# AsherJingkongChen/vlm-bridge-for-image-captioning

Hardware: NVIDIA B200
Metric: bridge fwd+bwd samples/sec (higher is better)
Workload: dtype bf16

## Files before the change

vlm-bridge-for-image-captioning_b200/csrc/attention.cu:

```cuda
#include <math.h>
#include <stdlib.h>
#include <string.h>

#include "common.cuh"
#include "launch.h"

namespace b200b {

int attention_fwd_tc(const b200b_attn_args* a, cudaStream_t stream, int* taken);
int attention_bwd_tc(const b200b_attn_args* a, const float* delta, cudaStream_t stream, int* taken);

struct AttnParams {
  const __nv_bfloat16* q; long long ldq;
  const __nv_bfloat16* k; long long ldk;
  const __nv_bfloat16* v; long long ldv;
  __nv_bfloat16* o; long long ldo;
  const __nv_bfloat16* d_o; long long lddo;
  __nv_bfloat16* dq; long long lddq;
  __nv_bfloat16* dk; long long lddk;
  __nv_bfloat16* dv; long long lddv;
  float* lse2;
  float* delta;
  __nv_bfloat16* p_scr;
  __nv_bfloat16* ds_scr;
  int B, H, Lq, Lk, Lkp;
  long long kv_bstride, kv_hstride;
  float scale, scale_log2;
  DropoutCfg drop;
  uint32_t drop_stream;
};

template <int HD>
struct AttnCfg {
  static constexpr int kBM = 64;
  static constexpr int kBN = (HD > 128) ? 32 : 64;
  static constexpr int kLd = HD + 8;
  static constexpr int kRowBytes = HD * 2;
  static constexpr int kQT = 32;
  static constexpr int kScrLd = 40;
  static constexpr size_t kFwdSmem = (size_t)(kBM + 4 * kBN) * kLd * 2;
  static constexpr size_t kBwdQSmem = (size_t)(2 * kBM + 4 * kBN) * kLd * 2;
  static constexpr size_t kBwdKVSmem = (size_t)2 * (2 * kQT * kScrLd + 2 * kQT * kLd) * 2;
};
// ... 468 lines not shown
    if (row0 < p.Lq) p.lse2[bh * p.Lq + row0] = m_run[0] + log2f(l_run[0]);
    if (row0 + 8 < p.Lq) p.lse2[bh * p.Lq + row0 + 8] = m_run[1] + log2f(l_run[1]);
  }
  {
    const float s0 = 1.0f / l_run[0], s1 = 1.0f / l_run[1];
    __nv_bfloat16* stage = Qs + (size_t)rg * 16 * kLd + half * (HD / 2);
#pragma unroll
    for (int n = 0; n < NH; ++n) {
      *reinterpret_cast<uint32_t*>(stage + (size_t)g * kLd + n * 8 + 2 * t4) = pack_bf16(o_acc[n][0] * s0, o_acc[n][1] * s0);
      *reinterpret_cast<uint32_t*>(stage + (size_t)(g + 8) * kLd + n * 8 + 2 * t4) =
          pack_bf16(o_acc[n][2] * s1, o_acc[n][3] * s1);
    }
    __syncwarp();
    const int rows_valid = max(0, min(16, nq - rg * 16));
    constexpr int kChunks = HD / 16;
    __nv_bfloat16* gdst = p.o + ((size_t)b * p.Lq + q0 + rg * 16) * p.ldo + (size_t)h * HD + half * (HD / 2);
    for (int idx = lane; idx < 16 * kChunks; idx += 32) {
      const int r = idx / kChunks, c = idx % kChunks;
      if (r < rows_valid)
        *reinterpret_cast<uint4*>(gdst + (size_t)r * p.ldo + c * 8) = *reinterpret_cast<const uint4*>(stage + (size_t)r * kLd + c * 8);
    }
  }
}

__global__ void attn_delta_kernel(const __nv_bfloat16* __restrict__ o, long long ldo,
                                  const __nv_bfloat16* __restrict__ d_o, long long lddo, float* __restrict__ delta,
                                  int B, int H, int Lq, int HD) {
  pdl_prologue();
  const int warp = threadIdx.x >> 5, lane = threadIdx.x & 31;
  const long long row = blockIdx.x;
  if (warp >= H) return;
  const uint32_t* po = reinterpret_cast<const uint32_t*>(o + row * ldo + (size_t)warp * HD);
  const uint32_t* pd = reinterpret_cast<const uint32_t*>(d_o + row * lddo + (size_t)warp * HD);
  float s = 0.f;
  for (int c = lane; c < HD / 2; c += 32) {
    const uint32_t a = po[c], d = pd[c];
    s += bf16_lo(a) * bf16_lo(d) + bf16_hi(a) * bf16_hi(d);
  }
  s = warp_sum(s);
  if (lane == 0) {
    const long long b = row / Lq, i = row % Lq;
    delta[((size_t)b * H + warp) * Lq + i] = s;
  }
}

template <int HD>
__global__ void __launch_bounds__(128) attn_bwd_q_kernel(const AttnParams p) {
  pdl_prologue();
  const DropoutCfg drop = dropout_resolve(p.drop);
  using Cfg = AttnCfg<HD>;
  constexpr int BN = Cfg::kBN, kLd = Cfg::kLd;
  extern __shared__ __align__(16) uint8_t smem_attn[];
  __nv_bfloat16* Qs = reinterpret_cast<__nv_bfloat16*>(smem_attn);
  __nv_bfloat16* dOs = Qs + (size_t)Cfg::kBM * kLd;
  __nv_bfloat16* Ks = dOs + (size_t)Cfg::kBM * kLd;
  __nv_bfloat16* Vs = Ks + (size_t)2 * BN * kLd;
  __shared__ __align__(8) uint64_t qbar, full_bar[2];

  const int warp = threadIdx.x >> 5, lane = threadIdx.x & 31;
  const int b = blockIdx.z, h = blockIdx.y, q0 = blockIdx.x * Cfg::kBM;
  const int nq = min(Cfg::kBM, p.Lq - q0);
  const int nt = (p.Lk + BN - 1) / BN;

  if (threadIdx.x == 0) {
    mbar_init(&qbar, 1);
    mbar_init(&full_bar[0], 1);
    mbar_init(&full_bar[1], 1);
    fence_barrier_init();
  }
  __syncthreads();
  if (warp == 0) {
    if (lane == 0) mbar_arrive_expect_tx(&qbar, (uint32_t)(2 * nq * Cfg::kRowBytes));
// ... 202 lines not shown
  launch_pdl(kPdlAttn, attn_fwd_kernel<HD>, grid, dim3(128), Cfg::kFwdSmem, stream, p);
  return check_launch("attn_fwd", stream);
}

static bool use_decode_kernel(const AttnParams& p) { return p.drop.thr == 0 && p.Lq <= 64; }

template <int HD, bool PACKED>
static int launch_decode(const AttnParams& p, cudaStream_t stream) {
  using Cfg = DecodeCfg<HD>;
  static bool attr_done = false;
  if (!attr_done) {
    int rc = set_smem(attn_decode_kernel<HD, PACKED>, Cfg::smem_bytes(2), "attn_decode");
    if (rc) return rc;
    attr_done = true;
  }
  const int nrg = (min(64, p.Lq) + 15) / 16;
  dim3 grid((p.Lq + 63) / 64, p.H, p.B);
  AttnParams pp = p;
#ifdef B200B_DIAG
  static const int dbg = [] { const char* e = getenv("B200B_DECODE_DEBUG"); return e ? atoi(e) : 0; }();
  if (dbg & 1) pp.Lkp = -1;
#endif
  launch_pdl(kPdlAttn, attn_decode_kernel<HD, PACKED>, grid, dim3(256), Cfg::smem_bytes(nrg), stream, pp);
  return check_launch(PACKED ? "attn_decode_packed" : "attn_decode", stream);
}

template <int HD>
static int launch_bwd(const AttnParams& p, cudaStream_t stream, const b200b_attn_args* a) {
  using Cfg = AttnCfg<HD>;
  int rc = set_smem(attn_bwd_q_kernel<HD>, Cfg::kBwdQSmem, "attn_bwd_q");
  if (rc) return rc;
  rc = set_smem(attn_bwd_kv_kernel<HD>, Cfg::kBwdKVSmem, "attn_bwd_kv");
  if (rc) return rc;
  const int delta_threads = 32 * p.H;
  launch_pdl(kPdlAttn, attn_delta_kernel, dim3(p.B * p.Lq), dim3(delta_threads), 0, stream, p.o, p.ldo, p.d_o, p.lddo, p.delta, p.B, p.H, p.Lq,
             HD);
  rc = check_launch("attn_delta", stream);
  if (rc) return rc;
  {
    int taken = 0;
    rc = attention_bwd_tc(a, p.delta, stream, &taken);
    if (taken) return rc;
  }
  dim3 gq((p.Lq + Cfg::kBM - 1) / Cfg::kBM, p.H, p.B);
  launch_pdl(kPdlAttn, attn_bwd_q_kernel<HD>, gq, dim3(128), Cfg::kBwdQSmem, stream, p);
  rc = check_launch("attn_bwd_q", stream);
  if (rc) return rc;
  dim3 gk((p.Lk + 31) / 32, p.H, p.B);
  launch_pdl(kPdlAttn, attn_bwd_kv_kernel<HD>, gk, dim3(128), Cfg::kBwdKVSmem, stream, p);
  return check_launch("attn_bwd_kv", stream);
}

static bool al16p(const void* p) { return (reinterpret_cast<uintptr_t>(p) & 15) == 0; }

static int validate_common(const b200b_attn_args* a, const char* what) {
  if (a == nullptr || !a->q || !a->k || !a->v || !a->o || !a->lse) {
    set_last_error("%s: null argument", what);
    return B200B_ERR_ARG;
  }
  if (a->batch <= 0 || a->heads <= 0 || a->heads > 32 || a->len_q <= 0 || a->len_k <= 0) {
    set_last_error("%s: bad sizes (batch=%d heads=%d len_q=%d len_k=%d)", what, a->batch, a->heads, a->len_q, a->len_k);
    return B200B_ERR_SHAPE;
  }
  if (a->head_dim != 64 && a->head_dim != 128 && a->head_dim != 288) {
    set_last_error("%s: head_dim %d not built (64, 128, 288)", what, a->head_dim);
    return B200B_ERR_SHAPE;
  }
  if (!al16p(a->q) || !al16p(a->k) || !al16p(a->v) || !al16p(a->o) || (a->ldq % 8) || (a->ldk % 8) || (a->ldv % 8) ||
      (a->ldo % 8)) {
    set_last_error("%s: q/k/v/o must be 16-byte aligned with row pitch multiple of 8 elements", what);
    return B200B_ERR_ALIGN;
  }
  if (!(a->dropout_p >= 0.0f && a->dropout_p < 1.0f)) {
    set_last_error("%s: dropout_p must be in [0,1)", what);
    return B200B_ERR_ARG;
  }
// ... 173 lines not shown
```

vlm-bridge-for-image-captioning_b200/csrc/attention_train_tc.cu:

```cuda
#include <stdlib.h>
#include <string.h>

#include "../../include/b200_bridge.h"
#include "common.cuh"
#include "launch.h"

namespace b200b {

struct FwdTcParams {
  __nv_bfloat16* o; long long ldo;
  float* lse2;
  int B, H, Lq, Lk, Lkp;
  float scale_log2;
  DropoutCfg drop;
  uint32_t drop_stream;
};

int attn_tc_mask();

constexpr int kFBM = 128;
constexpr int kFBN = 64;
constexpr int kFThreads = 192;

template <int HD>
// ... 235 lines not shown
  if (!attr_done) {
    cudaError_t e = cudaFuncSetAttribute(attn_fwd_tc_kernel<HD>, cudaFuncAttributeMaxDynamicSharedMemorySize,
                                         (int)Cfg::kSmemBytes);
    if (e != cudaSuccess) {
      set_last_error("attention_fwd (tcgen05): cudaFuncSetAttribute failed: %s", cudaGetErrorString(e));
      return (int)e;
    }
    attr_done = true;
  }
  CUtensorMap tq, tk, tv;
  int rc = make_tmap_heads_sw64(&tq, a->q, a->ldq, HD, a->heads, a->len_q, a->batch, kFBM);
  if (rc != B200B_OK) return rc;
  rc = make_tmap_heads_sw64(&tk, a->k, a->ldk, HD, a->heads, a->len_k, a->batch, kFBN);
  if (rc != B200B_OK) return rc;
  rc = make_tmap_heads_sw64(&tv, a->v, a->ldv, HD, a->heads, a->len_k, a->batch, kFBN);
  if (rc != B200B_OK) return rc;
  FwdTcParams p;
  p.o = reinterpret_cast<__nv_bfloat16*>(a->o);
  p.ldo = a->ldo;
  p.lse2 = a->lse;
  p.B = a->batch; p.H = a->heads; p.Lq = a->len_q; p.Lk = a->len_k; p.Lkp = (a->len_k + 7) & ~7;
  p.scale_log2 = 1.4426950408889634f / sqrtf((float)HD);
  p.drop_stream = a->dropout_stream;
  p.drop = make_dropout_cfg(a->dropout_p, a->seed, &p.drop_stream);
  dim3 grid((a->len_q + kFBM - 1) / kFBM, a->heads, a->batch);
  launch_pdl(kPdlAttn, attn_fwd_tc_kernel<HD>, grid, dim3(kFThreads), Cfg::kSmemBytes, stream, tq, tk, tv, p);
  return check_launch("attn_fwd_tc", stream);
}

struct BwdTcParams {
  __nv_bfloat16* dq; long long lddq;
  __nv_bfloat16* dk; long long lddk;
  __nv_bfloat16* dv; long long lddv;
  const float* lse2;
  const float* delta;
  int B, H, Lq, Lk, Lkp;
  float scale, scale_log2;
  DropoutCfg drop;
  uint32_t drop_stream;
};

template <int HD>
struct DqTcCfg {
  static constexpr int kChunks = HD / 32;
  static constexpr int kQBytes = kFBM * HD * 2;
  static constexpr int kTileBytes = kFBN * HD * 2;
  static constexpr int kN0 = HD > 256 ? 160 : HD;
  static constexpr int kN1 = HD - kN0;
  static constexpr int kSCol = 0;
  static constexpr int kDpCol = kFBN;
  static constexpr int kDsCol = 2 * kFBN;
  static constexpr int kDqCol = 3 * kFBN;
  static constexpr uint32_t kTmemCols = (kDqCol + HD) <= 256 ? 256 : 512;
  static constexpr size_t kSmemBytes = 2 * (size_t)kQBytes + 2 * (size_t)kTileBytes + 1024;
};

template <int HD>
__global__ void __launch_bounds__(kFThreads, 1)
attn_bwd_dq_tc_kernel(const __grid_constant__ CUtensorMap tm_q, const __grid_constant__ CUtensorMap tm_do,
                      const __grid_constant__ CUtensorMap tm_k, const __grid_constant__ CUtensorMap tm_v,
                      const BwdTcParams p) {
  using Cfg = DqTcCfg<HD>;
  extern __shared__ uint8_t smem_ftc_raw[];
  __shared__ __align__(8) uint64_t qdo_full, k_full, k_free, v_full, v_free, s_full, ds_full, dq_done[2];
  __shared__ uint32_t tmem_base_smem;

  const int warp = threadIdx.x >> 5, lane = threadIdx.x & 31;
  const int q0 = blockIdx.x * kFBM, h = blockIdx.y, b = blockIdx.z;
  const uint32_t s0 = (smem_u32(smem_ftc_raw) + 1023u) & ~1023u;
  const uint32_t q_tile = s0, do_tile = s0 + Cfg::kQBytes;
  const uint32_t k_tile = do_tile + Cfg::kQBytes, v_tile = k_tile + Cfg::kTileBytes;
  const int nt = (p.Lk + kFBN - 1) / kFBN;

  if (threadIdx.x == 0) {
    mbar_init(&qdo_full, 1);
    mbar_init(&k_full, 1);
    mbar_init(&k_free, 1);
    mbar_init(&v_full, 1);
    mbar_init(&v_free, 1);
    mbar_init(&s_full, 1);
    mbar_init(&ds_full, 4);
    mbar_init(&dq_done[0], 1);
    mbar_init(&dq_done[1], 1);
    fence_barrier_init();
  }
  if (warp == 0) {
    tmem_alloc(&tmem_base_smem, Cfg::kTmemCols);
    tmem_relinquish();
  }
  if (warp == 5 && lane == 0) {
    tma_prefetch_desc(&tm_q);
    tma_prefetch_desc(&tm_do);
    tma_prefetch_desc(&tm_k);
    tma_prefetch_desc(&tm_v);
  }
  pdl_launch_dependents();
  pdl_wait();
  tc_fence_before();
  __syncthreads();
  tc_fence_after();
  const uint32_t tmem_base = tmem_base_smem;
// ... 34 lines not shown
          umma_bf16(tmem_base + Cfg::kSCol, desc_sw64_kmajor(q_tile, kFBM, ks), desc_sw64_kmajor(k_tile, kFBN, ks), idesc_s,
                    ks > 0);
        mbar_wait(&v_full, ph);
        tc_fence_after();
#pragma unroll
        for (int ks = 0; ks < HD / 16; ++ks)
          umma_bf16(tmem_base + Cfg::kDpCol, desc_sw64_kmajor(do_tile, kFBM, ks), desc_sw64_kmajor(v_tile, kFBN, ks),
                    idesc_s, ks > 0);
        umma_commit(&s_full);
        umma_commit(&v_free);
        mbar_wait(&ds_full, ph);
        tc_fence_after();
        const uint32_t da = tmem_base + (uint32_t)(Cfg::kDsCol + (t & 1) * (kFBN / 2));
        const uint32_t dd = tmem_base + (uint32_t)Cfg::kDqCol;
#pragma unroll
        for (int kc = 0; kc < kFBN / 16; ++kc) {
          umma_bf16_tmem_a(dd, da + (uint32_t)(kc * 8), desc_sw64_mnmajor(k_tile, kFBN, 0, kc), idesc_q0, (t | kc) != 0);
          if constexpr (Cfg::kN1 > 0)
            umma_bf16_tmem_a(dd + (uint32_t)Cfg::kN0, da + (uint32_t)(kc * 8),
                             desc_sw64_mnmajor(k_tile, kFBN, Cfg::kN0 / 32, kc), idesc_q1, (t | kc) != 0);
        }
        umma_commit(&dq_done[t & 1]);
        umma_commit(&k_free);
      }
    }
  } else {
    const DropoutCfg drop = dropout_resolve(p.drop);
    const int row = warp * 32 + lane;
    const bool valid = q0 + row < p.Lq;
    const uint32_t lane_off = (uint32_t)(warp * 32) << 16;
    const size_t bh = (size_t)b * p.H + h;
    const uint64_t ridx = (bh * p.Lq + (uint64_t)(q0 + row)) * (uint64_t)p.Lkp;
    const float lse = valid ? p.lse2[bh * p.Lq + q0 + row] : 0.f;
    const float del = valid ? p.delta[bh * p.Lq + q0 + row] : 0.f;
    for (int t = 0; t < nt; ++t) {
      mbar_wait(&s_full, (uint32_t)(t & 1));
      tc_fence_after();
      if (t >= 2) mbar_wait(&dq_done[t & 1], (uint32_t)(((t >> 1) - 1) & 1));
      tc_fence_after();
#pragma unroll
      for (int half = 0; half < kFBN / 32; ++half) {
        uint32_t sv[2][16], dv[2][16];
#pragma unroll
        for (int g = 0; g < 2; ++g) {
          tmem_ld_32x32_x16(tmem_base + lane_off + (uint32_t)(Cfg::kSCol + half * 32 + g * 16), sv[g]);
          tmem_ld_32x32_x16(tmem_base + lane_off + (uint32_t)(Cfg::kDpCol + half * 32 + g * 16), dv[g]);
        }
        tmem_ld_wait();
        uint32_t w[16];
#pragma unroll
        for (int g = 0; g < 2; ++g) {
          float ds[16];
#pragma unroll
          for (int j8 = 0; j8 < 2; ++j8) {
            const int col0 = t * kFBN + half * 32 + g * 16 + j8 * 8;
            uint4 bits = make_uint4(0, 0, 0, 0);
            if (drop.thr != 0) bits = dropout_bits8(drop, p.drop_stream, (ridx + (uint64_t)col0) >> 3);
#pragma unroll
            for (int e = 0; e < 8; ++e) {
              const int j = j8 * 8 + e;
              const float pr = (col0 + e < p.Lk) ? exp2f(__uint_as_float(sv[g][j]) * p.scale_log2 - lse) : 0.f;
              float dpr = __uint_as_float(dv[g][j]);
              if (drop.thr != 0) dpr = dropout_keep(bits, e, drop.thr) ? dpr * drop.scale : 0.f;
              ds[j] = pr * (dpr - del);
            }
          }
#pragma unroll
// ... 18 lines not shown
      if (valid) {
        uint4 u[4];
        uint32_t* w = reinterpret_cast<uint32_t*>(u);
#pragma unroll
        for (int j = 0; j < 8; ++j) {
          w[j] = pack_bf16(__uint_as_float(v0[2 * j]) * p.scale, __uint_as_float(v0[2 * j + 1]) * p.scale);
          w[8 + j] = pack_bf16(__uint_as_float(v1[2 * j]) * p.scale, __uint_as_float(v1[2 * j + 1]) * p.scale);
        }
#pragma unroll
        for (int j = 0; j < 4; ++j) *reinterpret_cast<uint4*>(dst + c0 + j * 8) = u[j];
      }
    }
  }
  tc_fence_before();
  __syncthreads();
  if (warp == 0) tmem_dealloc(tmem_base, Cfg::kTmemCols);
}

template <int HD>
struct DkvTcCfg {
  static constexpr int kChunks = HD / 32;
  static constexpr int kTileBytes = kFBM * HD * 2;
  static constexpr int kN0 = HD > 256 ? 160 : HD;
  static constexpr int kN1 = HD - kN0;
  static constexpr int kStCol = 0;
  static constexpr int kDptCol = 128;
  static constexpr int kOutCol = 192;
  static constexpr uint32_t kTmemCols = 512;
  static constexpr size_t kSmemBytes = 3 * (size_t)kTileBytes + 1024;
  static_assert(kOutCol + HD <= 512, "head dim");
};

template <int HD>
__global__ void __launch_bounds__(kFThreads, 1)
attn_bwd_dkv_tc_kernel(const __grid_constant__ CUtensorMap tm_q, const __grid_constant__ CUtensorMap tm_do,
                       const __grid_constant__ CUtensorMap tm_k, const __grid_constant__ CUtensorMap tm_v,
                       const BwdTcParams p, const int blocks_per_cta) {
  using Cfg = DkvTcCfg<HD>;
  extern __shared__ uint8_t smem_ftc_raw[];
  __shared__ __align__(8) uint64_t q_full, do_full, k_full, v_full, k_free, v_free, st_full, dpt_full, pds_full, dv_done,
      dv_drained, dk_done, dk_drained;
  __shared__ uint32_t tmem_base_smem;
  __shared__ float lse_s[kFBM], del_s[kFBM];

  const int warp = threadIdx.x >> 5, lane = threadIdx.x & 31;
  const int h = blockIdx.y, b = blockIdx.z;
  const int nkb = (p.Lk + kFBM - 1) / kFBM;
  const int jb0 = blockIdx.x * blocks_per_cta;
  const int nit = min(blocks_per_cta, nkb - jb0);
  const uint32_t s0 = (smem_u32(smem_ftc_raw) + 1023u) & ~1023u;
  const uint32_t a_tile = s0, q_tile = s0 + Cfg::kTileBytes, do_tile = q_tile + Cfg::kTileBytes;
  const size_t bh = (size_t)b * p.H + h;

  if (threadIdx.x == 0) {
    mbar_init(&q_full, 1);
    mbar_init(&do_full, 1);
    mbar_init(&k_full, 1);
    mbar_init(&v_full, 1);
    mbar_init(&k_free, 1);
    mbar_init(&v_free, 1);
    mbar_init(&st_full, 1);
    mbar_init(&dpt_full, 1);
    mbar_init(&pds_full, 4);
    mbar_init(&dv_done, 1);
    mbar_init(&dv_drained, 4);
    mbar_init(&dk_done, 1);
    mbar_init(&dk_drained, 4);
    fence_barrier_init();
  }
  if (warp == 0) {
    tmem_alloc(&tmem_base_smem, Cfg::kTmemCols);
    tmem_relinquish();
  }
  if (warp == 5 && lane == 0) {
    tma_prefetch_desc(&tm_q);
    tma_prefetch_desc(&tm_do);
    tma_prefetch_desc(&tm_k);
    tma_prefetch_desc(&tm_v);
  }
  pdl_launch_dependents();
  pdl_wait();
  if (threadIdx.x < kFBM) {
    const bool ok = (int)threadIdx.x < p.Lq;
    lse_s[threadIdx.x] = ok ? p.lse2[bh * p.Lq + threadIdx.x] : 0.f;
    del_s[threadIdx.x] = ok ? p.delta[bh * p.Lq + threadIdx.x] : 0.f;
  }
  tc_fence_before();
  __syncthreads();
  tc_fence_after();
  const uint32_t tmem_base = tmem_base_smem;

  if (warp == 5) {
    if (lane == 0) {
      mbar_arrive_expect_tx(&q_full, Cfg::kTileBytes);
#pragma unroll
      for (int c = 0; c < Cfg::kChunks; ++c)
        tma_load_4d(q_tile + (uint32_t)c * kFBM * 64, &tm_q, smem_u32(&q_full), c * 32, h, 0, b);
      for (int it = 0; it < nit; ++it) {
        const int j0 = (jb0 + it) * kFBM;
        const uint32_t prev = (uint32_t)((it - 1) & 1);
        if (it >= 1) mbar_wait(&v_free, prev);
        mbar_arrive_expect_tx(&k_full, Cfg::kTileBytes);
#pragma unroll
        for (int c = 0; c < Cfg::kChunks; ++c)
          tma_load_4d(a_tile + (uint32_t)c * kFBM * 64, &tm_k, smem_u32(&k_full), c * 32, h, j0, b);
        if (it == 0) {
          mbar_arrive_expect_tx(&do_full, Cfg::kTileBytes);
#pragma unroll
          for (int c = 0; c < Cfg::kChunks; ++c)
            tma_load_4d(do_tile + (uint32_t)c * kFBM * 64, &tm_do, smem_u32(&do_full), c * 32, h, 0, b);
        }
        mbar_wait(&k_free, (uint32_t)(it & 1));
        mbar_arrive_expect_tx(&v_full, Cfg::kTileBytes);
#pragma unroll
        for (int c = 0; c < Cfg::kChunks; ++c)
          tma_load_4d(a_tile + (uint32_t)c * kFBM * 64, &tm_v, smem_u32(&v_full), c * 32, h, j0, b);
      }
    }
  } else if (warp == 4) {
    if (lane == 0) {
      constexpr uint32_t idesc_s = umma_idesc_bf16(kFBM, kFBM, false, false);
      constexpr uint32_t idesc_o0 = umma_idesc_bf16(kFBM, Cfg::kN0, false, true);
      constexpr uint32_t idesc_o1 = umma_idesc_bf16(kFBM, Cfg::kN1 > 0 ? Cfg::kN1 : 16, false, true);
      const uint32_t od = tmem_base + (uint32_t)Cfg::kOutCol;
      mbar_wait(&q_full, 0);
      for (int it = 0; it < nit; ++it) {
        const uint32_t ph = (uint32_t)(it & 1);
        mbar_wait(&k_full, ph);
        tc_fence_after();
#pragma unroll
        for (int ks = 0; ks < HD / 16; ++ks)
          umma_bf16(tmem_base + Cfg::kStCol, desc_sw64_kmajor(a_tile, kFBM, ks), desc_sw64_kmajor(q_tile, kFBM, ks), idesc_s,
                    ks > 0);
        umma_commit(&st_full);
        umma_commit(&k_free);
        if (it == 0) mbar_wait(&do_full, 0);
        mbar_wait(&v_full, ph);
        tc_fence_after();
#pragma unroll
        for (int ks = 0; ks < HD / 16; ++ks)
          umma_bf16(tmem_base + Cfg::kDptCol, desc_sw64_kmajor(a_tile, kFBM, ks), desc_sw64_kmajor(do_tile, kFBM, ks),
                    idesc_s, ks > 0);
        umma_commit(&dpt_full);
        umma_commit(&v_free);
        mbar_wait(&pds_full, ph);
        if (it >= 1) mbar_wait(&dk_drained, (uint32_t)((it - 1) & 1));
        tc_fence_after();
#pragma unroll
        for (int kc = 0; kc < kFBM / 16; ++kc) {
          umma_bf16_tmem_a(od, tmem_base + (uint32_t)(Cfg::kStCol + kc * 8), desc_sw64_mnmajor(do_tile, kFBM, 0, kc),
                           idesc_o0, kc != 0);
          if constexpr (Cfg::kN1 > 0)
            umma_bf16_tmem_a(od + (uint32_t)Cfg::kN0, tmem_base + (uint32_t)(Cfg::kStCol + kc * 8),
                             desc_sw64_mnmajor(do_tile, kFBM, Cfg::kN0 / 32, kc), idesc_o1, kc != 0);
        }
        umma_commit(&dv_done);
        mbar_wait(&dv_drained, ph);
        tc_fence_after();
#pragma unroll
        for (int kc = 0; kc < kFBM / 16; ++kc) {
          umma_bf16_tmem_a(od, tmem_base + (uint32_t)(Cfg::kDptCol + kc * 8), desc_sw64_mnmajor(q_tile, kFBM, 0, kc),
                           idesc_o0, kc != 0);
          if constexpr (Cfg::kN1 > 0)
            umma_bf16_tmem_a(od + (uint32_t)Cfg::kN0, tmem_base + (uint32_t)(Cfg::kDptCol + kc * 8),
                             desc_sw64_mnmajor(q_tile, kFBM, Cfg::kN0 / 32, kc), idesc_o1, kc != 0);
        }
        umma_commit(&dk_done);
      }
    }
  } else {
    const DropoutCfg drop = dropout_resolve(p.drop);
    const int row = warp * 32 + lane;
    const uint32_t lane_off = (uint32_t)(warp * 32) << 16;
    for (int it = 0; it < nit; ++it) {
      const uint32_t ph = (uint32_t)(it & 1);
      const int j0 = (jb0 + it) * kFBM;
      const int key = j0 + row;
      const bool key_ok = key < p.Lk;
      const uint64_t kgrp = (uint64_t)((j0 + warp * 32) >> 3) + (uint64_t)(lane >> 3);
      mbar_wait(&st_full, ph);
      mbar_wait(&dpt_full, ph);
      tc_fence_after();
#pragma unroll 1
      for (int c = 0; c < kFBM / 32; ++c) {
        uint32_t sv[2][16], dv[2][16];
#pragma unroll
        for (int g = 0; g < 2; ++g) {
          tmem_ld_32x32_x16(tmem_base + lane_off + (uint32_t)(Cfg::kStCol + c * 32 + g * 16), sv[g]);
          tmem_ld_32x32_x16(tmem_base + lane_off + (uint32_t)(Cfg::kDptCol + c * 32 + g * 16), dv[g]);
        }
        tmem_ld_wait();
        uint4 bits[4];
        if (drop.thr != 0) {
#pragma unroll
          for (int r = 0; r < 4; ++r) {
            const uint64_t qi = (uint64_t)(c * 32 + r * 8 + (lane & 7));
            bits[r] = dropout_bits8(drop, p.drop_stream, ((bh * p.Lq + qi) * (uint64_t)p.Lkp >> 3) + kgrp);
          }
        }
        uint32_t wp[16], wd[16];
#pragma unroll
        for (int g = 0; g < 2; ++g) {
          float pv[16], dsv[16];
#pragma unroll
          for (int j = 0; j < 16; ++j) {
            const int qi = c * 32 + g * 16 + j;
// ... 39 lines not shown
          if (key_ok) {
            uint4 u[4];
            uint32_t* w = reinterpret_cast<uint32_t*>(u);
#pragma unroll
            for (int j = 0; j < 8; ++j) {
              w[j] = pack_bf16(__uint_as_float(v0[2 * j]) * mul, __uint_as_float(v0[2 * j + 1]) * mul);
              w[8 + j] = pack_bf16(__uint_as_float(v1[2 * j]) * mul, __uint_as_float(v1[2 * j + 1]) * mul);
            }
#pragma unroll
            for (int j = 0; j < 4; ++j) *reinterpret_cast<uint4*>(dst + c0 + j * 8) = u[j];
          }
        }
      };
      mbar_wait(&dv_done, ph);
      tc_fence_after();
      drain(p.dv, p.lddv, 1.0f);
      tc_fence_before();
      __syncwarp();
      if (lane == 0) mbar_arrive(&dv_drained);
      mbar_wait(&dk_done, ph);
      tc_fence_after();
      drain(p.dk, p.lddk, p.scale);
      tc_fence_before();
      __syncwarp();
      if (lane == 0) mbar_arrive(&dk_drained);
    }
  }
  tc_fence_before();
  __syncthreads();
  if (warp == 0) tmem_dealloc(tmem_base, Cfg::kTmemCols);
}

template <int HD>
static int launch_bwd_tc(const b200b_attn_args* a, const float* delta, cudaStream_t stream) {
  static bool attr_done = false;
  if (!attr_done) {
    cudaError_t e = cudaFuncSetAttribute(attn_bwd_dq_tc_kernel<HD>, cudaFuncAttributeMaxDynamicSharedMemorySize,
                                         (int)DqTcCfg<HD>::kSmemBytes);
    if (e == cudaSuccess)
      e = cudaFuncSetAttribute(attn_bwd_dkv_tc_kernel<HD>, cudaFuncAttributeMaxDynamicSharedMemorySize,
                               (int)DkvTcCfg<HD>::kSmemBytes);
    if (e != cudaSuccess) {
      set_last_error("attention_bwd (tcgen05): cudaFuncSetAttribute failed: %s", cudaGetErrorString(e));
      return (int)e;
    }
    attr_done = true;
  }
  BwdTcParams p;
  p.dq = reinterpret_cast<__nv_bfloat16*>(a->dq); p.lddq = a->lddq;
  p.dk = reinterpret_cast<__nv_bfloat16*>(a->dk); p.lddk = a->lddk;
  p.dv = reinterpret_cast<__nv_bfloat16*>(a->dv); p.lddv = a->lddv;
  p.lse2 = a->lse;
  p.delta = delta;
  p.B = a->batch; p.H = a->heads; p.Lq = a->len_q; p.Lk = a->len_k; p.Lkp = (a->len_k + 7) & ~7;
  p.scale = 1.0f / sqrtf((float)HD);
  p.scale_log2 = p.scale * 1.4426950408889634f;
  p.drop_stream = a->dropout_stream;
  p.drop = make_dropout_cfg(a->dropout_p, a->seed, &p.drop_stream);
  CUtensorMap tq, td, tk, tv;
  int rc;
  if ((rc = make_tmap_heads_sw64(&tq, a->q, a->ldq, HD, a->heads, a->len_q, a->batch, kFBM)) != B200B_OK) return rc;
  if ((rc = make_tmap_heads_sw64(&td, a->d_o, a->lddo, HD, a->heads, a->len_q, a->batch, kFBM)) != B200B_OK) return rc;
  if ((rc = make_tmap_heads_sw64(&tk, a->k, a->ldk, HD, a->heads, a->len_k, a->batch, kFBN)) != B200B_OK) return rc;
  if ((rc = make_tmap_heads_sw64(&tv, a->v, a->ldv, HD, a->heads, a->len_k, a->batch, kFBN)) != B200B_OK) return rc;
  dim3 gq((a->len_q + kFBM - 1) / kFBM, a->heads, a->batch);
  launch_pdl(kPdlAttn, attn_bwd_dq_tc_kernel<HD>, gq, dim3(kFThreads), DqTcCfg<HD>::kSmemBytes, stream, tq, td, tk, tv, p);
  if ((rc = check_launch("attn_bwd_dq_tc", stream)) != B200B_OK) return rc;
  if ((rc = make_tmap_heads_sw64(&tk, a->k, a->ldk, HD, a->heads, a->len_k, a->batch, kFBM)) != B200B_OK) return rc;
  if ((rc = make_tmap_heads_sw64(&tv, a->v, a->ldv, HD, a->heads, a->len_k, a->batch, kFBM)) != B200B_OK) return rc;
  int num_sms = 0;
  if ((rc = device_sm_count(&num_sms)) != B200B_OK) return rc;
  const int nkb = (a->len_k + kFBM - 1) / kFBM;
  const long long items = (long long)nkb * a->heads * a->batch;
  int bpc = (int)((items + 2LL * num_sms - 1) / (2LL * num_sms));
  if (bpc < 1) bpc = 1;
  const int ctas_per_head = (nkb + bpc - 1) / bpc;
  bpc = (nkb + ctas_per_head - 1) / ctas_per_head;
  dim3 gk((nkb + bpc - 1) / bpc, a->heads, a->batch);
  launch_pdl(kPdlAttn, attn_bwd_dkv_tc_kernel<HD>, gk, dim3(kFThreads), DkvTcCfg<HD>::kSmemBytes, stream, tq, td, tk, tv, p,
             bpc);
  return check_launch("attn_bwd_dkv_tc", stream);
}

int attention_bwd_tc(const b200b_attn_args* a, const float* delta, cudaStream_t stream, int* taken) {
  *taken = 0;
  if (!(attn_tc_mask() & 2) || a->len_q > kFBM) return B200B_OK;
  const uintptr_t al = reinterpret_cast<uintptr_t>(a->q) | reinterpret_cast<uintptr_t>(a->k) | reinterpret_cast<uintptr_t>(a->v) |
                       reinterpret_cast<uintptr_t>(a->d_o) | reinterpret_cast<uintptr_t>(a->dq) |
                       reinterpret_cast<uintptr_t>(a->dk) | reinterpret_cast<uintptr_t>(a->dv);
  if ((al & 15) || (a->ldq % 8) || (a->ldk % 8) || (a->ldv % 8) || (a->lddo % 8) || (a->lddq % 8) || (a->lddk % 8) ||
      (a->lddv % 8))
    return B200B_OK;
  int rc;
  switch (a->head_dim) {
    case 64: rc = launch_bwd_tc<64>(a, delta, stream); break;
    case 128: rc = launch_bwd_tc<128>(a, delta, stream); break;
    case 288: rc = launch_bwd_tc<288>(a, delta, stream); break;
    default: return B200B_OK;
  }
  *taken = 1;
  return rc;
}

static int g_attn_tc = -1;
int attn_tc_mask() {
  if (g_attn_tc < 0) {
    const char* e = getenv("B200B_ATTN_TC");
    g_attn_tc = e ? atoi(e) : 3;
  }
  return g_attn_tc;
}

int attention_fwd_tc(const b200b_attn_args* a, cudaStream_t stream, int* taken) {
  *taken = 0;
  if (!(attn_tc_mask() & 1)) return B200B_OK;
  const uintptr_t al = reinterpret_cast<uintptr_t>(a->q) | reinterpret_cast<uintptr_t>(a->k) | reinterpret_cast<uintptr_t>(a->v) |
                       reinterpret_cast<uintptr_t>(a->o);
  if ((al & 15) || (a->ldq % 8) || (a->ldk % 8) || (a->ldv % 8) || (a->ldo % 8)) return B200B_OK;
  int rc;
  switch (a->head_dim) {
    case 64: rc = launch_fwd_tc<64>(a, stream); break;
    case 128: rc = launch_fwd_tc<128>(a, stream); break;
    case 288: rc = launch_fwd_tc<288>(a, stream); break;
    default: return B200B_OK;
  }
  *taken = 1;
  return rc;
}

}
// ... 7 lines not shown
```

vlm-bridge-for-image-captioning_b200/csrc/common.cuh:

```cuda
#pragma once

#include <cuda.h>
#include <cuda_bf16.h>
#include <cuda_runtime.h>
#include <stdint.h>
#include <stdio.h>

#include "../../include/b200_bridge.h"

namespace b200b {

__device__ __forceinline__ uint32_t smem_u32(const void* p) {
  return static_cast<uint32_t>(__cvta_generic_to_shared(p));
}
__device__ __forceinline__ int lane_id() { return threadIdx.x & 31; }

__device__ __forceinline__ uint32_t pack_bf16(float lo, float hi) {
  __nv_bfloat162 v = __floats2bfloat162_rn(lo, hi);
  return *reinterpret_cast<uint32_t*>(&v);
}
__device__ __forceinline__ float bf16_round(float x) {
  return __bfloat162float(__float2bfloat16_rn(x));
}
__device__ __forceinline__ float bf16_lo(uint32_t v) { return __uint_as_float(v << 16); }
__device__ __forceinline__ float bf16_hi(uint32_t v) { return __uint_as_float(v & 0xffff0000u); }

__device__ __forceinline__ float warp_sum(float v) {
#pragma unroll
  for (int o = 16; o > 0; o >>= 1) v += __shfl_xor_sync(0xffffffffu, v, o);
  return v;
}
__device__ __forceinline__ float warp_max(float v) {
#pragma unroll
  for (int o = 16; o > 0; o >>= 1) v = fmaxf(v, __shfl_xor_sync(0xffffffffu, v, o));
  return v;
}

__device__ __forceinline__ float rcp_approx(float x) {
  float r;
  asm("rcp.approx.ftz.f32 %0, %1;" : "=f"(r) : "f"(x));
  return r;
}
__device__ __forceinline__ float ex2_approx(float x) {
  float r;
  asm("ex2.approx.ftz.f32 %0, %1;" : "=f"(r) : "f"(x));
  return r;
}
__device__ __forceinline__ float normal_cdf(float x, float* gauss) {
  const float z = fabsf(x) * 0.70710678118654752440f;
  const float t = rcp_approx(fmaf(0.3275911f, z, 1.0f));
  float poly = fmaf(t, 1.061405429f, -1.453152027f);
  poly = fmaf(poly, t, 1.421413741f);
  poly = fmaf(poly, t, -0.284496736f);
  poly = fmaf(poly, t, 0.254829592f);
  poly *= t;
  const float e = ex2_approx(-1.4426950408889634f * z * z);
  *gauss = e;
  const float half_erfc = 0.5f * poly * e;
  return x >= 0.0f ? 1.0f - half_erfc : half_erfc;
}
__device__ __forceinline__ float gelu_erf(float x) {
  float g;
  return x * normal_cdf(x, &g);
// ... 429 lines not shown
```

Measured before the change: 5022.

## Fuse attention backward dQ and dKV tcgen05 kernels and compute delta in-kernel

Merges the separate dQ and dKV tensor-core backward kernels into one launch whose blocks pick a role by index, and removes the separate delta kernel by having each CTA compute delta rows from O and dO itself. It also moves the dk_drained wait earlier in the dKV MMA issue sequence. The aim is fewer launches and dependency gaps and letting dQ and dKV work run concurrently. In exchange, delta is computed redundantly across CTAs, and both roles share the larger shared-memory footprint.

```diff
diff --git a/vlm-bridge-for-image-captioning_b200/csrc/attention.cu b/vlm-bridge-for-image-captioning_b200/csrc/attention.cu
--- a/vlm-bridge-for-image-captioning_b200/csrc/attention.cu
+++ b/vlm-bridge-for-image-captioning_b200/csrc/attention.cu
@@ -8,7 +8,7 @@
 namespace b200b {
 
 int attention_fwd_tc(const b200b_attn_args* a, cudaStream_t stream, int* taken);
-int attention_bwd_tc(const b200b_attn_args* a, const float* delta, cudaStream_t stream, int* taken);
+int attention_bwd_tc(const b200b_attn_args* a, cudaStream_t stream, int* taken);
 
 struct AttnParams {
   const __nv_bfloat16* q; long long ldq;
@@ -543,12 +543,7 @@
   if (warp >= H) return;
   const uint32_t* po = reinterpret_cast<const uint32_t*>(o + row * ldo + (size_t)warp * HD);
   const uint32_t* pd = reinterpret_cast<const uint32_t*>(d_o + row * lddo + (size_t)warp * HD);
-  float s = 0.f;
-  for (int c = lane; c < HD / 2; c += 32) {
-    const uint32_t a = po[c], d = pd[c];
-    s += bf16_lo(a) * bf16_lo(d) + bf16_hi(a) * bf16_hi(d);
-  }
-  s = warp_sum(s);
+  const float s = warp_sum(bf16_row_dot_lane(po, pd, HD / 2, lane));
   if (lane == 0) {
     const long long b = row / Lq, i = row % Lq;
     delta[((size_t)b * H + warp) * Lq + i] = s;
@@ -817,16 +812,16 @@
   if (rc) return rc;
   rc = set_smem(attn_bwd_kv_kernel<HD>, Cfg::kBwdKVSmem, "attn_bwd_kv");
   if (rc) return rc;
+  {
+    int taken = 0;
+    rc = attention_bwd_tc(a, stream, &taken);
+    if (taken) return rc;
+  }
   const int delta_threads = 32 * p.H;
   launch_pdl(kPdlAttn, attn_delta_kernel, dim3(p.B * p.Lq), dim3(delta_threads), 0, stream, p.o, p.ldo, p.d_o, p.lddo, p.delta, p.B, p.H, p.Lq,
              HD);
   rc = check_launch("attn_delta", stream);
   if (rc) return rc;
-  {
-    int taken = 0;
-    rc = attention_bwd_tc(a, p.delta, stream, &taken);
-    if (taken) return rc;
-  }
   dim3 gq((p.Lq + Cfg::kBM - 1) / Cfg::kBM, p.H, p.B);
   launch_pdl(kPdlAttn, attn_bwd_q_kernel<HD>, gq, dim3(128), Cfg::kBwdQSmem, stream, p);
   rc = check_launch("attn_bwd_q", stream);
diff --git a/vlm-bridge-for-image-captioning_b200/csrc/attention_train_tc.cu b/vlm-bridge-for-image-captioning_b200/csrc/attention_train_tc.cu
--- a/vlm-bridge-for-image-captioning_b200/csrc/attention_train_tc.cu
+++ b/vlm-bridge-for-image-captioning_b200/csrc/attention_train_tc.cu
@@ -291,13 +291,49 @@
   __nv_bfloat16* dq; long long lddq;
   __nv_bfloat16* dk; long long lddk;
   __nv_bfloat16* dv; long long lddv;
+  const __nv_bfloat16* o; long long ldo;
+  const __nv_bfloat16* d_o; long long lddo;
   const float* lse2;
-  const float* delta;
   int B, H, Lq, Lk, Lkp;
   float scale, scale_log2;
   DropoutCfg drop;
   uint32_t drop_stream;
 };
+
+template <int HD>
+__device__ __forceinline__ void delta_rows_tc(const BwdTcParams& p, int r0, int h, int b, float* del_s, int warp,
+                                              int lane) {
+  constexpr int kPairs = HD / 2, kIters = (kPairs + 31) / 32;
+  constexpr int kRows = kIters == 1 ? 32 : kIters == 2 ? 16 : 8;
+#pragma unroll 1
+  for (int r = warp * 32; r < warp * 32 + 32; r += kRows) {
+    uint32_t x[kRows][kIters], y[kRows][kIters];
+#pragma unroll
+    for (int u = 0; u < kRows; ++u) {
+      const int qi = r0 + r + u;
+      const size_t tok = (size_t)b * p.Lq + (qi < p.Lq ? qi : 0);
+      const uint32_t* po = reinterpret_cast<const uint32_t*>(p.o + tok * p.ldo + (size_t)h * HD);
+      const uint32_t* pd = reinterpret_cast<const uint32_t*>(p.d_o + tok * p.lddo + (size_t)h * HD);
+#pragma unroll
+      for (int i = 0; i < kIters; ++i) {
+        const int c = lane + 32 * i;
+        const bool ok = qi < p.Lq && c < kPairs;
+        x[u][i] = ok ? po[c] : 0u;
+        y[u][i] = ok ? pd[c] : 0u;
+      }
+    }
+#pragma unroll
+    for (int u = 0; u < kRows; ++u) {
+      float s = 0.f;
+#pragma unroll
+      for (int i = 0; i < kIters; ++i)
+        if (lane + 32 * i < kPairs) s += bf16_pair_dot(x[u][i], y[u][i]);
+      s = warp_sum(s);
+      if (lane == 0) del_s[r + u] = r0 + r + u < p.Lq ? s : 0.f;
+    }
+  }
+  asm volatile("bar.sync 1, 128;" ::: "memory");
+}
 
 template <int HD>
 struct DqTcCfg {
@@ -315,17 +351,16 @@
 };
 
 template <int HD>
-__global__ void __launch_bounds__(kFThreads, 1)
-attn_bwd_dq_tc_kernel(const __grid_constant__ CUtensorMap tm_q, const __grid_constant__ CUtensorMap tm_do,
-                      const __grid_constant__ CUtensorMap tm_k, const __grid_constant__ CUtensorMap tm_v,
-                      const BwdTcParams p) {
+__device__ __forceinline__ void attn_bwd_dq_role(const CUtensorMap& tm_q, const CUtensorMap& tm_do,
+                                                 const CUtensorMap& tm_k, const CUtensorMap& tm_v, const BwdTcParams& p,
+                                                 const int q0, const int h, const int b) {
   using Cfg = DqTcCfg<HD>;
   extern __shared__ uint8_t smem_ftc_raw[];
   __shared__ __align__(8) uint64_t qdo_full, k_full, k_free, v_full, v_free, s_full, ds_full, dq_done[2];
   __shared__ uint32_t tmem_base_smem;
+  __shared__ float del_s[kFBM];
 
   const int warp = threadIdx.x >> 5, lane = threadIdx.x & 31;
-  const int q0 = blockIdx.x * kFBM, h = blockIdx.y, b = blockIdx.z;
   const uint32_t s0 = (smem_u32(smem_ftc_raw) + 1023u) & ~1023u;
   const uint32_t q_tile = s0, do_tile = s0 + Cfg::kQBytes;
   const uint32_t k_tile = do_tile + Cfg::kQBytes, v_tile = k_tile + Cfg::kTileBytes;
@@ -426,7 +461,8 @@
     const size_t bh = (size_t)b * p.H + h;
     const uint64_t ridx = (bh * p.Lq + (uint64_t)(q0 + row)) * (uint64_t)p.Lkp;
     const float lse = valid ? p.lse2[bh * p.Lq + q0 + row] : 0.f;
-    const float del = valid ? p.delta[bh * p.Lq + q0 + row] : 0.f;
+    delta_rows_tc<HD>(p, q0, h, b, del_s, warp, lane);
+    const float del = del_s[row];
     for (int t = 0; t < nt; ++t) {
       mbar_wait(&s_full, (uint32_t)(t & 1));
       tc_fence_after();
@@ -511,10 +547,9 @@
 };
 
 template <int HD>
-__global__ void __launch_bounds__(kFThreads, 1)
-attn_bwd_dkv_tc_kernel(const __grid_constant__ CUtensorMap tm_q, const __grid_constant__ CUtensorMap tm_do,
-                       const __grid_constant__ CUtensorMap tm_k, const __grid_constant__ CUtensorMap tm_v,
-                       const BwdTcParams p, const int blocks_per_cta) {
+__device__ __forceinline__ void attn_bwd_dkv_role(const CUtensorMap& tm_q, const CUtensorMap& tm_do,
+                                                  const CUtensorMap& tm_k, const CUtensorMap& tm_v, const BwdTcParams& p,
+                                                  const int jb0, const int blocks_per_cta, const int h, const int b) {
   using Cfg = DkvTcCfg<HD>;
   extern __shared__ uint8_t smem_ftc_raw[];
   __shared__ __align__(8) uint64_t q_full, do_full, k_full, v_full, k_free, v_free, st_full, dpt_full, pds_full, dv_done,
@@ -523,9 +558,7 @@
   __shared__ float lse_s[kFBM], del_s[kFBM];
 
   const int warp = threadIdx.x >> 5, lane = threadIdx.x & 31;
-  const int h = blockIdx.y, b = blockIdx.z;
   const int nkb = (p.Lk + kFBM - 1) / kFBM;
-  const int jb0 = blockIdx.x * blocks_per_cta;
   const int nit = min(blocks_per_cta, nkb - jb0);
   const uint32_t s0 = (smem_u32(smem_ftc_raw) + 1023u) & ~1023u;
   const uint32_t a_tile = s0, q_tile = s0 + Cfg::kTileBytes, do_tile = q_tile + Cfg::kTileBytes;
@@ -562,7 +595,6 @@
   if (threadIdx.x < kFBM) {
     const bool ok = (int)threadIdx.x < p.Lq;
     lse_s[threadIdx.x] = ok ? p.lse2[bh * p.Lq + threadIdx.x] : 0.f;
-    del_s[threadIdx.x] = ok ? p.delta[bh * p.Lq + threadIdx.x] : 0.f;
   }
   tc_fence_before();
   __syncthreads();
@@ -615,6 +647,7 @@
         umma_commit(&k_free);
         if (it == 0) mbar_wait(&do_full, 0);
         mbar_wait(&v_full, ph);
+        if (it >= 1) mbar_wait(&dk_drained, (uint32_t)((it - 1) & 1));
         tc_fence_after();
 #pragma unroll
         for (int ks = 0; ks < HD / 16; ++ks)
@@ -623,7 +656,6 @@
         umma_commit(&dpt_full);
         umma_commit(&v_free);
         mbar_wait(&pds_full, ph);
-        if (it >= 1) mbar_wait(&dk_drained, (uint32_t)((it - 1) & 1));
         tc_fence_after();
 #pragma unroll
         for (int kc = 0; kc < kFBM / 16; ++kc) {
@@ -651,6 +683,7 @@
     const DropoutCfg drop = dropout_resolve(p.drop);
     const int row = warp * 32 + lane;
     const uint32_t lane_off = (uint32_t)(warp * 32) << 16;
+    delta_rows_tc<HD>(p, 0, h, b, del_s, warp, lane);
     for (int it = 0; it < nit; ++it) {
       const uint32_t ph = (uint32_t)(it & 1);
       const int j0 = (jb0 + it) * kFBM;
@@ -756,14 +789,29 @@
 }
 
 template <int HD>
-static int launch_bwd_tc(const b200b_attn_args* a, const float* delta, cudaStream_t stream) {
+__global__ void __launch_bounds__(kFThreads, 1)
+attn_bwd_tc_kernel(const __grid_constant__ CUtensorMap tm_q, const __grid_constant__ CUtensorMap tm_do,
+                   const __grid_constant__ CUtensorMap tm_k64, const __grid_constant__ CUtensorMap tm_v64,
+                   const __grid_constant__ CUtensorMap tm_k128, const __grid_constant__ CUtensorMap tm_v128,
+                   const BwdTcParams p, const int q_items, const int kv_ctas_per_head, const int blocks_per_cta) {
+  const int nqb = (p.Lq + kFBM - 1) / kFBM;
+  int item = blockIdx.x;
+  if (item < q_items) {
+    attn_bwd_dq_role<HD>(tm_q, tm_do, tm_k64, tm_v64, p, (item % nqb) * kFBM, (item / nqb) % p.H, item / (nqb * p.H));
+  } else {
+    item -= q_items;
+    attn_bwd_dkv_role<HD>(tm_q, tm_do, tm_k128, tm_v128, p, (item % kv_ctas_per_head) * blocks_per_cta, blocks_per_cta,
+                          (item / kv_ctas_per_head) % p.H, item / (kv_ctas_per_head * p.H));
+  }
+}
+
+template <int HD>
+static int launch_bwd_tc(const b200b_attn_args* a, cudaStream_t stream) {
+  constexpr size_t kSmem = DqTcCfg<HD>::kSmemBytes > DkvTcCfg<HD>::kSmemBytes ? DqTcCfg<HD>::kSmemBytes
+                                                                                : DkvTcCfg<HD>::kSmemBytes;
   static bool attr_done = false;
   if (!attr_done) {
-    cudaError_t e = cudaFuncSetAttribute(attn_bwd_dq_tc_kernel<HD>, cudaFuncAttributeMaxDynamicSharedMemorySize,
-                                         (int)DqTcCfg<HD>::kSmemBytes);
-    if (e == cudaSuccess)
-      e = cudaFuncSetAttribute(attn_bwd_dkv_tc_kernel<HD>, cudaFuncAttributeMaxDynamicSharedMemorySize,
-                               (int)DkvTcCfg<HD>::kSmemBytes);
+    cudaError_t e = cudaFuncSetAttribute(attn_bwd_tc_kernel<HD>, cudaFuncAttributeMaxDynamicSharedMemorySize, (int)kSmem);
     if (e != cudaSuccess) {
       set_last_error("attention_bwd (tcgen05): cudaFuncSetAttribute failed: %s", cudaGetErrorString(e));
       return (int)e;
@@ -774,24 +822,22 @@
   p.dq = reinterpret_cast<__nv_bfloat16*>(a->dq); p.lddq = a->lddq;
   p.dk = reinterpret_cast<__nv_bfloat16*>(a->dk); p.lddk = a->lddk;
   p.dv = reinterpret_cast<__nv_bfloat16*>(a->dv); p.lddv = a->lddv;
+  p.o = reinterpret_cast<const __nv_bfloat16*>(a->o); p.ldo = a->ldo;
+  p.d_o = reinterpret_cast<const __nv_bfloat16*>(a->d_o); p.lddo = a->lddo;
   p.lse2 = a->lse;
-  p.delta = delta;
   p.B = a->batch; p.H = a->heads; p.Lq = a->len_q; p.Lk = a->len_k; p.Lkp = (a->len_k + 7) & ~7;
   p.scale = 1.0f / sqrtf((float)HD);
   p.scale_log2 = p.scale * 1.4426950408889634f;
   p.drop_stream = a->dropout_stream;
   p.drop = make_dropout_cfg(a->dropout_p, a->seed, &p.drop_stream);
-  CUtensorMap tq, td, tk, tv;
+  CUtensorMap tq, td, tk64, tv64, tk128, tv128;
   int rc;
   if ((rc = make_tmap_heads_sw64(&tq, a->q, a->ldq, HD, a->heads, a->len_q, a->batch, kFBM)) != B200B_OK) return rc;
   if ((rc = make_tmap_heads_sw64(&td, a->d_o, a->lddo, HD, a->heads, a->len_q, a->batch, kFBM)) != B200B_OK) return rc;
-  if ((rc = make_tmap_heads_sw64(&tk, a->k, a->ldk, HD, a->heads, a->len_k, a->batch, kFBN)) != B200B_OK) return rc;
-  if ((rc = make_tmap_heads_sw64(&tv, a->v, a->ldv, HD, a->heads, a->len_k, a->batch, kFBN)) != B200B_OK) return rc;
-  dim3 gq((a->len_q + kFBM - 1) / kFBM, a->heads, a->batch);
-  launch_pdl(kPdlAttn, attn_bwd_dq_tc_kernel<HD>, gq, dim3(kFThreads), DqTcCfg<HD>::kSmemBytes, stream, tq, td, tk, tv, p);
-  if ((rc = check_launch("attn_bwd_dq_tc", stream)) != B200B_OK) return rc;
-  if ((rc = make_tmap_heads_sw64(&tk, a->k, a->ldk, HD, a->heads, a->len_k, a->batch, kFBM)) != B200B_OK) return rc;
-  if ((rc = make_tmap_heads_sw64(&tv, a->v, a->ldv, HD, a->heads, a->len_k, a->batch, kFBM)) != B200B_OK) return rc;
+  if ((rc = make_tmap_heads_sw64(&tk64, a->k, a->ldk, HD, a->heads, a->len_k, a->batch, kFBN)) != B200B_OK) return rc;
+  if ((rc = make_tmap_heads_sw64(&tv64, a->v, a->ldv, HD, a->heads, a->len_k, a->batch, kFBN)) != B200B_OK) return rc;
+  if ((rc = make_tmap_heads_sw64(&tk128, a->k, a->ldk, HD, a->heads, a->len_k, a->batch, kFBM)) != B200B_OK) return rc;
+  if ((rc = make_tmap_heads_sw64(&tv128, a->v, a->ldv, HD, a->heads, a->len_k, a->batch, kFBM)) != B200B_OK) return rc;
   int num_sms = 0;
   if ((rc = device_sm_count(&num_sms)) != B200B_OK) return rc;
   const int nkb = (a->len_k + kFBM - 1) / kFBM;
@@ -800,13 +846,15 @@
   if (bpc < 1) bpc = 1;
   const int ctas_per_head = (nkb + bpc - 1) / bpc;
   bpc = (nkb + ctas_per_head - 1) / ctas_per_head;
-  dim3 gk((nkb + bpc - 1) / bpc, a->heads, a->batch);
-  launch_pdl(kPdlAttn, attn_bwd_dkv_tc_kernel<HD>, gk, dim3(kFThreads), DkvTcCfg<HD>::kSmemBytes, stream, tq, td, tk, tv, p,
-             bpc);
-  return check_launch("attn_bwd_dkv_tc", stream);
-}
-
-int attention_bwd_tc(const b200b_attn_args* a, const float* delta, cudaStream_t stream, int* taken) {
+  const int q_items = (a->len_q + kFBM - 1) / kFBM * a->heads * a->batch;
+  const int kv_ctas_per_head = (nkb + bpc - 1) / bpc;
+  const dim3 grid(q_items + kv_ctas_per_head * a->heads * a->batch);
+  launch_pdl(kPdlAttn, attn_bwd_tc_kernel<HD>, grid, dim3(kFThreads), kSmem, stream, tq, td, tk64, tv64, tk128, tv128, p,
+             q_items, kv_ctas_per_head, bpc);
+  return check_launch("attn_bwd_tc", stream);
+}
+
+int attention_bwd_tc(const b200b_attn_args* a, cudaStream_t stream, int* taken) {
   *taken = 0;
   if (!(attn_tc_mask() & 2) || a->len_q > kFBM) return B200B_OK;
   const uintptr_t al = reinterpret_cast<uintptr_t>(a->q) | reinterpret_cast<uintptr_t>(a->k) | reinterpret_cast<uintptr_t>(a->v) |
@@ -817,9 +865,9 @@
     return B200B_OK;
   int rc;
   switch (a->head_dim) {
-    case 64: rc = launch_bwd_tc<64>(a, delta, stream); break;
-    case 128: rc = launch_bwd_tc<128>(a, delta, stream); break;
-    case 288: rc = launch_bwd_tc<288>(a, delta, stream); break;
+    case 64: rc = launch_bwd_tc<64>(a, stream); break;
+    case 128: rc = launch_bwd_tc<128>(a, stream); break;
+    case 288: rc = launch_bwd_tc<288>(a, stream); break;
     default: return B200B_OK;
   }
   *taken = 1;
diff --git a/vlm-bridge-for-image-captioning_b200/csrc/common.cuh b/vlm-bridge-for-image-captioning_b200/csrc/common.cuh
--- a/vlm-bridge-for-image-captioning_b200/csrc/common.cuh
+++ b/vlm-bridge-for-image-captioning_b200/csrc/common.cuh
@@ -29,6 +29,14 @@
 #pragma unroll
   for (int o = 16; o > 0; o >>= 1) v += __shfl_xor_sync(0xffffffffu, v, o);
   return v;
+}
+__device__ __forceinline__ float bf16_pair_dot(uint32_t x, uint32_t y) {
+  return bf16_lo(x) * bf16_lo(y) + bf16_hi(x) * bf16_hi(y);
+}
+__device__ __forceinline__ float bf16_row_dot_lane(const uint32_t* a, const uint32_t* b, int n2, int lane) {
+  float s = 0.f;
+  for (int c = lane; c < n2; c += 32) s += bf16_pair_dot(a[c], b[c]);
+  return s;
 }
 __device__ __forceinline__ float warp_max(float v) {
 #pragma unroll
```

Measured after the change: 5107, median of 6. +1.7%, better.
